# olsonanl/signature_kmers

Measured on AMD Instinct MI355X. Metric: k-mers/sec (extract+hash+count) at 1/2/4/8 GPUs; achieved HBM GB/s %, higher is better.
Workload: dtype u8

## Files before the change

### include/skm.h

```cpp
#ifndef SKM_H
#define SKM_H

#include <stddef.h>
#include <stdint.h>

#ifdef __cplusplus
extern "C" {
#endif

#define SKM_OK 0
#define SKM_E_ARG -1
#define SKM_E_HIP -2
#define SKM_E_OOM -3
#define SKM_E_IO -4
#define SKM_E_COMM -5
#define SKM_E_STATE -6

#define SKM_UNDEFINED_FUNCTION 0xFFFFu

typedef struct skm_stored_kmer_data {
    uint16_t avg_from_end;
    uint16_t function_index;
    uint16_t mean;
    uint16_t median;
// ... 50 lines not shown
int skm_build_prepare(skm_build* b);
int skm_build_run(skm_build* b);
int skm_build_last_timings(skm_build* b, float* ms, int cap);
int skm_build_set_kernel_timing(skm_build* b, int enable, const char* only);
int skm_build_kernel_timings(skm_build* b, char* names, size_t names_cap, float* ms, uint64_t* launches, int cap);
int skm_build_counters(skm_build* b, uint64_t* out, int cap);
typedef struct skm_transport {
    void* ctx;
    int (*alltoallv)(void* ctx, const void* send, const uint64_t* scnt, const uint64_t* soff, void* recv,
                     const uint64_t* rcnt, const uint64_t* roff);
    int (*allreduce)(void* ctx, void* data, uint64_t count, int op);
    int (*allgatherv)(void* ctx, const void* send, void* recv, const uint64_t* bytes_per_rank);
} skm_transport;
int skm_build_set_transport(skm_build* b, const skm_transport* tp);
int skm_debug_exchange_plan(const skm_transport* tp, int rank, int world, uint32_t nb1, const uint64_t* bucket_starts,
                            uint64_t* recv_off, uint64_t* recv_cnt, uint64_t* vstart);
int skm_debug_transport_check(const skm_transport* tp, int rank, int world);

int skm_build_set_option(skm_build* b, const char* name, int64_t value);
int skm_build_debug_stamps(skm_build* b, int enable, uint64_t* out, int cap);
int skm_build_debug_jobs(skm_build* b, uint32_t* out, int cap);
int skm_build_debug_overflow(skm_build* b, uint32_t* out, int cap);
int skm_build_debug_front(skm_build* b, uint64_t* out, int cap);
int skm_build_debug_pass_windows(skm_build* b, uint64_t* out, int cap);
int skm_debug_chain_bench(uint32_t n, uint32_t njobs, int mode, float* ms);
int skm_debug_chain_eval(const uint32_t* samples, uint32_t n, int mode, double* median, double* var);
int skm_debug_div_check(uint64_t nm, uint32_t per, uint64_t* mismatches);
int skm_build_finish(skm_build* b, skm_kept* out);
int skm_build_finish_slice(skm_build* b, int slice_bits, uint32_t slice, skm_kept* out);
int skm_build_signature_flags(skm_build* b, uint8_t* out, uint64_t cap);
void skm_kept_free(skm_kept* k);
void skm_build_destroy(skm_build* b);

int skm_comm_unique_id(uint8_t id[128]);
int skm_build_set_comm(skm_build* b, const uint8_t id[128]);
int skm_build_group_run(skm_build* const* bs, int n);

typedef struct skm_db skm_db;

int skm_db_open(skm_db** out, const char* mph_path, const char* dat_path, int device);
int skm_db_open_mem(skm_db** out, const uint8_t* mph, size_t mph_len, const uint8_t* dat,
                    size_t dat_len, int device);
int skm_db_open_kept(skm_db** out, const uint64_t* keys, const skm_stored_kmer_data* data, size_t n, int device);

typedef struct skm_kept_db_opts {
    uint32_t load_pct;
// ... 188 lines not shown
```

### signature_kmers_amd/__init__.py

```python
from __future__ import annotations

import ctypes as C
import os
from dataclasses import dataclass

import numpy as np

__all__ = [
    "SkmError", "lib", "K", "UNDEFINED_FUNCTION", "STORED_DTYPE", "CALL_DTYPE",
    "SignatureBuilder", "KeptKmers", "CmphKmerDb", "FunctionCaller", "mph_build",
    "kmer_to_str", "str_to_kmer", "keys_from_strings", "device_count", "MatrixDistance", "SeqIdMap",
    "matrix_tile_rows", "KeptKmerDb", "DeviceKeptKmerDb", "kept_db_plan", "kept_slot",
]

K = 8
UNDEFINED_FUNCTION = 0xFFFF
_HERE = os.path.dirname(os.path.abspath(__file__))
LIB_PATH = os.environ.get("SKM_LIB_PATH") or os.path.join(_HERE, "libskm.so")

STORED_DTYPE = np.dtype([("avg_from_end", "<u2"), ("function_index", "<u2"), ("mean", "<u2"),
                         ("median", "<u2"), ("var", "<u2")])
CALL_DTYPE = np.dtype([("start", "<u4"), ("end", "<u4"), ("count", "<i4"), ("function_index", "<u2"),
                       ("pad", "<u2"), ("protein_length_median", "<u4"),
                       ("protein_length_med_avg_dev", "<f4")])
# ... 86 lines not shown
    "skm_version": (C.c_char_p, []),
    "skm_device_count": (C.c_int, [C.POINTER(C.c_int)]),
    "skm_device_mem_info": (C.c_int, [C.c_int, C.POINTER(C.c_uint64), C.POINTER(C.c_uint64)]),
    "skm_build_create": (C.c_int, [C.POINTER(_P), C.POINTER(C.c_int), C.c_int, C.POINTER(_BuildOpts)]),
    "skm_build_add_batch": (C.c_int, [_P, _P, _P, _P, _P, _P, C.c_size_t]),
    "skm_build_prepare": (C.c_int, [_P]),
    "skm_build_run": (C.c_int, [_P]),
    "skm_build_last_timings": (C.c_int, [_P, C.POINTER(C.c_float), C.c_int]),
    "skm_build_set_kernel_timing": (C.c_int, [_P, C.c_int, C.c_char_p]),
    "skm_build_kernel_timings": (C.c_int, [_P, C.c_char_p, C.c_size_t, C.POINTER(C.c_float), C.POINTER(C.c_uint64),
                                           C.c_int]),
    "skm_build_finish": (C.c_int, [_P, C.POINTER(_Kept)]),
    "skm_build_finish_slice": (C.c_int, [_P, C.c_int, C.c_uint32, C.POINTER(_Kept)]),
    "skm_build_signature_flags": (C.c_int, [_P, _P, C.c_uint64]),
    "skm_build_set_option": (C.c_int, [_P, C.c_char_p, C.c_int64]),
    "skm_build_set_transport": (C.c_int, [_P, C.POINTER(_Transport)]),
    "skm_debug_exchange_plan": (C.c_int, [C.POINTER(_Transport), C.c_int, C.c_int, C.c_uint32, _P, _P, _P, _P]),
    "skm_debug_transport_check": (C.c_int, [C.POINTER(_Transport), C.c_int, C.c_int]),
    "skm_build_counters": (C.c_int, [_P, C.POINTER(C.c_uint64), C.c_int]),
    "skm_build_reserve": (C.c_int, [_P, C.c_uint64, C.c_uint64]),
    "skm_build_debug_jobs": (C.c_int, [_P, C.POINTER(C.c_uint32), C.c_int]),
    "skm_build_debug_overflow": (C.c_int, [_P, C.POINTER(C.c_uint32), C.c_int]),
    "skm_build_debug_front": (C.c_int, [_P, C.POINTER(C.c_uint64), C.c_int]),
    "skm_build_debug_pass_windows": (C.c_int, [_P, C.POINTER(C.c_uint64), C.c_int]),
    "skm_debug_chain_bench": (C.c_int, [C.c_uint32, C.c_uint32, C.c_int, C.POINTER(C.c_float)]),
    "skm_debug_chain_eval": (C.c_int, [_P, C.c_uint32, C.c_int, C.POINTER(C.c_double), C.POINTER(C.c_double)]),
    "skm_build_debug_stamps": (C.c_int, [_P, C.c_int, C.POINTER(C.c_uint64), C.c_int]),
    "skm_kept_free": (None, [C.POINTER(_Kept)]),
    "skm_build_destroy": (None, [_P]),
    "skm_comm_unique_id": (C.c_int, [_P]),
    "skm_build_set_comm": (C.c_int, [_P, _P]),
    "skm_build_group_run": (C.c_int, [C.POINTER(_P), C.c_int]),
    "skm_debug_div_check": (C.c_int, [C.c_uint64, C.c_uint32, C.POINTER(C.c_uint64)]),
    "skm_db_open": (C.c_int, [C.POINTER(_P), C.c_char_p, C.c_char_p, C.c_int]),
    "skm_db_open_mem": (C.c_int, [C.POINTER(_P), _P, C.c_size_t, _P, C.c_size_t, C.c_int]),
    "skm_db_open_kept": (C.c_int, [C.POINTER(_P), _P, _P, C.c_size_t, C.c_int]),
    "skm_build_kept_db": (C.c_int, [_P, C.POINTER(_KeptDbOpts), C.POINTER(_P)]),
    "skm_kept_db_plan": (C.c_int, [C.c_uint64, C.POINTER(_KeptDbOpts), C.POINTER(C.c_uint64), C.POINTER(C.c_uint64)]),
    "skm_debug_kept_slot": (C.c_int, [C.c_uint64, C.c_uint64, C.POINTER(C.c_uint64)]),
    "skm_build_mph_db": (C.c_int, [_P, C.POINTER(_MphDbOpts), C.POINTER(_P), C.c_void_p]),
    "skm_mph_db_plan": (C.c_int, [C.c_uint64, C.POINTER(C.c_uint64)]),
    "skm_build_write_final_kmers": (C.c_int, [_P, C.c_char_p, C.POINTER(_FinalKmersStats)]),
    "skm_build_stats": (C.c_int, [_P, C.POINTER(_Kept)]),
    "skm_final_kmers_info": (C.c_int, [C.POINTER(C.c_uint32)]),
    "skm_debug_final_kmers_host": (C.c_int, [_P, _P, C.c_size_t, _P, C.c_size_t, C.POINTER(C.c_uint64)]),
    "skm_db_lookup_fm": (C.c_int, [_P, _P, C.c_size_t, _P]),
# ... 245 lines not shown
                 "free_after_prepare", "recs_rot", "overflow_light_subbuckets", "overflow_light_elements",
                 "groupby_tasks", "groupby_batches"]
        return {names[i]: int(v[i]) for i in range(n)}

    def debug_jobs(self, k: int = 64) -> list:
        v = (C.c_uint32 * k)()
        _check(lib().skm_build_debug_jobs(self._h, v, k))
        return [int(x) for x in v]

    def debug_overflow(self, k: int = 4096) -> list:
        v = (C.c_uint32 * k)()
        n = lib().skm_build_debug_overflow(self._h, v, k)
        return [int(x) for x in v[:min(max(n, 0), k)]]

    def debug_front(self) -> dict:
        names = ["rp", "sel_wg", "sel_span", "emit_g", "pf_span", "pf_nwg", "nwg", "span", "pass_bits",
                 "owner_bits", "b1_bits"]
        v = (C.c_uint64 * len(names))()
        n = lib().skm_build_debug_front(self._h, v, len(names))
        _check(min(n, 0))
        assert n == len(names), n
        return {names[i]: int(v[i]) for i in range(n)}

    def debug_pass_windows(self) -> list:
        v = (C.c_uint64 * 64)()
        n = lib().skm_build_debug_pass_windows(self._h, v, 64)
        _check(min(n, 0))
        return [int(x) for x in v[:n]]

    def debug_stamps(self, enable: bool) -> list:
        v = (C.c_uint64 * 32)()
        _check(lib().skm_build_debug_stamps(self._h, 1 if enable else 0, v, 32))
        return [int(x) for x in v]

    def finish(self) -> KeptKmers:
        k = _Kept()
        _check(lib().skm_build_finish(self._h, C.byref(k)))
        return self._kept(k)

    def finish_slice(self, slice_bits: int, slice_: int) -> KeptKmers:
        k = _Kept()
        _check(lib().skm_build_finish_slice(self._h, int(slice_bits), int(slice_), C.byref(k)))
        return self._kept(k)

    def signature_flags(self) -> np.ndarray:
        n = self.counters()["sequences"]
# ... 824 lines not shown
```

### signature_kmers_amd/csrc/skm_build.hip

```cpp
#include <fcntl.h>
#include <hip/hip_runtime.h>
#include <unistd.h>

#include <algorithm>
#include <cerrno>
#include <type_traits>
#include <chrono>
#include <cmath>
#include <cstdio>
#include <cstdlib>
#include <cstring>
#include <deque>
#include <memory>
#include <numeric>
#include <string>
#include <thread>
#include <vector>

#include "skm_common.h"
#include "skm_keptdb.h"
#include "skm_mphdb.h"
#include "skm_pool.h"
#include "skm_output.h"
#include "skm_util.h"
// ... 1682 lines not shown
                    if (q == j) f = off[j]++;
                s_out[f] = ((uint64_t)(16u * lane + (uint32_t)t) << KEY_BITS) | hs[t];
            }
        }
        wave_sync();
        for (uint32_t j = lane; j < qa[G]; j += 64) {
            uint32_t q = 0;
#pragma unroll
            for (uint32_t k = 1; k < G; ++k) q += j >= qa[k] ? 1u : 0u;
            uint64_t o = 0;
#pragma unroll
            for (uint32_t k = 0; k < G; ++k)
                if (q == k) o = run[k] + (j - qa[k]);
            const uint64_t v = s_out[j];
            if (o < cap) pos[(uint64_t)q * cap + o] = ((t0 - a + (v >> KEY_BITS)) << KEY_BITS) | (v & H43_MASK);
        }
#pragma unroll
        for (uint32_t q = 0; q < G; ++q) run[q] += qa[q + 1] - qa[q];
        wave_sync();
    }
}

constexpr uint32_t PH_THREADS = 512;
__global__ __launch_bounds__(PH_THREADS) void k_pass_hist(const uint64_t* __restrict__ pos, uint64_t cap,
                                                          const unsigned long long* __restrict__ npos, uint32_t NB,
                                                          int rem_bits, uint32_t* __restrict__ hist) {
    extern __shared__ uint32_t s_h[];
    const uint32_t q = blockIdx.y;
    for (uint32_t k = threadIdx.x; k < NB; k += PH_THREADS) s_h[k] = 0;
    __syncthreads();
    const uint64_t n = min((uint64_t)npos[q], cap);
    const uint64_t* p = pos + (uint64_t)q * cap;
    constexpr uint32_t U = 4;
    for (uint64_t j0 = (uint64_t)blockIdx.x * PH_THREADS * U; j0 < n; j0 += (uint64_t)gridDim.x * PH_THREADS * U) {
        uint64_t v[U];
#pragma unroll
        for (uint32_t u = 0; u < U; ++u) {
            const uint64_t j = j0 + u * PH_THREADS + threadIdx.x;
            v[u] = j < n ? p[j] : ~0ull;
        }
#pragma unroll
        for (uint32_t u = 0; u < U; ++u)
            if (v[u] != ~0ull) atomicAdd(&s_h[(uint32_t)((v[u] & H43_MASK) >> rem_bits) & (NB - 1)], 1u);
    }
    __syncthreads();
    uint32_t* hq = hist + (uint64_t)q * NB;
    for (uint32_t k = threadIdx.x; k < NB; k += PH_THREADS)
        if (s_h[k]) atomicAdd(&hq[k], s_h[k]);
}

__global__ __launch_bounds__(EX_THREADS) void k_extract(ExtractArgs X) {
    const uint8_t* __restrict__ res = X.res;
    const uint64_t rp = X.rp, span = X.span;
    extern __shared__ uint32_t s_cnt[];
    const int nbits = X.owner_bits + X.b1_bits;
    const uint32_t NB = 1u << nbits;
    const int rem_bits = KEY_BITS - nbits;
    const uint32_t wg = blockIdx.x;
    for (uint32_t b = threadIdx.x; b < NB; b += blockDim.x) s_cnt[b] = 0u;
    __syncthreads();
    const uint64_t begin = (uint64_t)wg * span;
    const uint64_t end = min(begin + span, rp);
    for (uint64_t base = begin + (uint64_t)threadIdx.x * EX_POS_PER_THREAD; base < end;
         base += (uint64_t)blockDim.x * EX_POS_PER_THREAD) {
        const uint4 v0 = *reinterpret_cast<const uint4*>(res + base);
        const uint4 v1 = *reinterpret_cast<const uint4*>(res + base + 16);
        const uint32_t w[8] = {v0.x, v0.y, v0.z, v0.w, v1.x, v1.y, v1.z, v1.w};
        uint32_t code[24];
// ... 4 lines not shown
            uint32_t cd = residue_code(c);
            valid |= (cd < 40u ? 1u : 0u) << j;
            code[j] = cd < 40u ? cd : 0u;
        }
        uint64_t k = 0;
#pragma unroll
        for (int j = 0; j < 8; ++j) k = k * 40u + code[j];
        constexpr uint64_t P7 = 6553600000000ull / 40u;
#pragma unroll
        for (int t = 0; t < EX_POS_PER_THREAD; ++t) {
            if (t > 0) k = (k - (uint64_t)code[t - 1] * P7) * 40u + code[t + 7];
            const uint64_t p = base + t;
            if (((valid >> t) & 0xFFu) == 0xFFu && p < end) {
                const uint64_t h = mix43(k);
                atomicAdd(&s_cnt[(uint32_t)(h >> rem_bits)], 1u);
            }
        }
    }
    __syncthreads();
    for (uint32_t b = threadIdx.x; b < NB; b += blockDim.x) X.hist[(uint64_t)wg * NB + b] = s_cnt[b];
}

constexpr int SC_ROUND = 4096;
constexpr int SC_L0_BITS = 6;
constexpr int SC_POS = SC_ROUND / EX_THREADS;
constexpr uint64_t SC_SLICE = 65536;

constexpr uint32_t CUR_STRIDE = 16;

template <int R>
struct StageLdsT {
    uint64_t hi[R];
    uint64_t lo[R];
    uint8_t dst[R];
    uint32_t cnt[128];
    uint32_t off[129];
    unsigned long long base[128];
    uint32_t wave[48];
};
using StageLds = StageLdsT<SC_ROUND>;
constexpr int SC_ROUND_HALF = SC_ROUND / 2;

__device__ __forceinline__ uint32_t agg_rank(uint32_t* cnt, uint32_t d, bool v) {
    const uint32_t lane = threadIdx.x & 63u;
    const uint64_t act = __ballot(v);
    if (act == 0) return 0u;
    const uint32_t l0 = (uint32_t)__ffsll((long long)act) - 1u;
// ... 104 lines not shown
        for (int t = 0; t < SC_POS; ++t)
            if ((ok >> t) & 1u) {
                const uint32_t slot = L.off[l0[t]] + rk[t];
                L.hi[slot] = eh[t];
                L.lo[slot] = el[t];
                L.dst[slot] = (uint8_t)l0[t];
            }
        __syncthreads();
        for (uint32_t j = threadIdx.x; j < tot; j += blockDim.x) {
            const uint32_t d = L.dst[j];
            const uint64_t o = L.base[d] + (j - L.off[d]);
            out_hi[o] = L.hi[j];
            out_lo[o] = L.lo[j];
        }
        __syncthreads();
    }
}

template <int R, int MINB>
__global__ __launch_bounds__(EX_THREADS, MINB) void k_extract_stage_pos(ExtractArgs X, const uint64_t* __restrict__ pos,
                                                                        const unsigned long long* __restrict__ np,
                                                                        const uint64_t* __restrict__ sel, uint32_t nrows,
                                                                        uint64_t sel_span,
                                                                        unsigned long long* __restrict__ cur0,
                                                                        uint64_t* __restrict__ out_hi,
                                                                        uint64_t* __restrict__ out_lo) {
    constexpr int SC_POS = R / EX_THREADS;
    const uint64_t n = min((uint64_t)*np, X.pos_cap);
    __shared__ StageLdsT<R> L;
    const int nbits = X.owner_bits + X.b1_bits;
    const uint32_t NB = 1u << nbits;
    const int rem_bits = KEY_BITS - X.pass_bits - nbits;
    const uint64_t rem_mask = (1ull << rem_bits) - 1;
    const int l0_shift = nbits - SC_L0_BITS;
    const uint64_t begin = (uint64_t)blockIdx.x * X.span, end = min(begin + X.span, n);
    uint32_t s = 0xFFFFFFFFu;
    SeqMeta m{};
    uint32_t row = 0;
    {
        const uint64_t j0 = begin + (uint64_t)threadIdx.x * SC_POS;
        uint32_t lo = 0, hi = nrows;
        while (hi - lo > 1) {
            const uint32_t mid = (lo + hi) >> 1;
            if (sel[mid] <= j0)
                lo = mid;
            else
                hi = mid;
        }
        row = lo;
    }
    uint64_t row_end = sel[row + 1];
    uint64_t nxt[SC_POS];
#pragma unroll
    for (int t = 0; t < SC_POS; ++t) {
        const uint64_t j = begin + (uint64_t)threadIdx.x * SC_POS + t;
        nxt[t] = j < end ? pos[j] : ~0ull;
    }
    for (uint64_t base = begin; base < end; base += R) {
        if (threadIdx.x < 128) L.cnt[threadIdx.x] = 0;
        __syncthreads();
        uint64_t ent[SC_POS];
#pragma unroll
        for (int t = 0; t < SC_POS; ++t) ent[t] = nxt[t];
#pragma unroll
        for (int t = 0; t < SC_POS; ++t) {
            const uint64_t j = base + R + (uint64_t)threadIdx.x * SC_POS + t;
            nxt[t] = j < end ? pos[j] : ~0ull;
        }
        uint64_t eh[SC_POS], el[SC_POS];
        uint32_t rk[SC_POS], l0[SC_POS];
#pragma unroll
        for (int t = 0; t < SC_POS; ++t) {
            eh[t] = el[t] = 0;
            rk[t] = l0[t] = 0;
            if (ent[t] != ~0ull) {
                const uint64_t j = base + (uint64_t)threadIdx.x * SC_POS + t;
                while (j >= row_end) row_end = sel[++row + 1];
                const uint64_t p = (uint64_t)row * sel_span + (ent[t] >> KEY_BITS);
                if (s == 0xFFFFFFFFu || p < m.pstart || p > m.pstart + m.len) {
                    s = X.blk2seq[p >> 6];
                    m = X.meta[s];
                }
                while (p > m.pstart + m.len) m = X.meta[++s];
                const uint64_t h = ent[t] & H43_MASK;
                const uint32_t bucket = (uint32_t)(h >> rem_bits) & (NB - 1);
                const uint64_t route = (uint64_t)((uint32_t)(h >> (KEY_BITS - X.pass_bits)) ^ X.pass_id) << rem_bits;
                make_elem((h & rem_mask) | route, X.s_base + s, (uint32_t)(p - m.pstart), m, eh[t], el[t]);
                el[t] = (el[t] & ~0xFFFFull) | bucket;
                l0[t] = bucket >> l0_shift;
            }
        }
#pragma unroll
        for (int t = 0; t < SC_POS; ++t) rk[t] = agg_rank(L.cnt, l0[t], ent[t] != ~0ull);
        __syncthreads();
        const uint32_t tot = stage_reserve(L, 1u << SC_L0_BITS, cur0, 0);
#pragma unroll
        for (int t = 0; t < SC_POS; ++t)
            if (ent[t] != ~0ull) {
                const uint32_t slot = L.off[l0[t]] + rk[t];
                L.hi[slot] = eh[t];
                L.lo[slot] = el[t];
                L.dst[slot] = (uint8_t)l0[t];
            }
        __syncthreads();
        for (uint32_t j = threadIdx.x; j < tot; j += blockDim.x) {
            const uint32_t d = L.dst[j];
            const uint64_t o = L.base[d] + (j - L.off[d]);
            out_hi[o] = L.hi[j];
            out_lo[o] = L.lo[j];
        }
        __syncthreads();
    }
}

__global__ void k_stage_init(const uint64_t* __restrict__ bstart, uint32_t NB, int l0_shift,
                             unsigned long long* __restrict__ cur0, unsigned long long* __restrict__ cur1,
                             uint32_t* __restrict__ slice_base) {
    const uint32_t t = blockIdx.x * blockDim.x + threadIdx.x;
    if (t < NB) cur1[(uint64_t)t * CUR_STRIDE] = bstart[t];
    if (blockIdx.x == 0) {
        __shared__ uint32_t s_n[(1 << SC_L0_BITS) + 1];
        const uint32_t n0 = 1u << SC_L0_BITS;
        if (threadIdx.x < n0) {
            const uint64_t a = bstart[(uint64_t)threadIdx.x << l0_shift];
            const uint64_t e = bstart[(uint64_t)(threadIdx.x + 1) << l0_shift];
            cur0[threadIdx.x * CUR_STRIDE] = a;
            s_n[threadIdx.x] = (uint32_t)((e - a + SC_SLICE - 1) / SC_SLICE);
        }
        __syncthreads();
        if (threadIdx.x == 0) {
            uint32_t acc = 0;
            for (uint32_t b = 0; b < n0; ++b) {
                slice_base[b] = acc;
                acc += s_n[b];
            }
// ... 972 lines not shown
    const uint64_t thr = 2 * (total / max(nb, 1u));
    const uint32_t per = (nb + blockDim.x - 1) / blockDim.x;
    const uint32_t b0 = min(nb, threadIdx.x * per), b1 = min(nb, b0 + per);
    uint32_t loc = 0;
    for (uint32_t b = b0; b < b1; ++b) loc += bstart[b + 1] - bstart[b] > thr ? 1u : 0u;
    uint32_t nbig;
    uint32_t pos = wg_exclusive_scan(loc, s_wave, nbig);
    uint32_t sp = b0 - pos;
    for (uint32_t b = b0; b < b1; ++b) {
        if (bstart[b + 1] - bstart[b] > thr)
            order[pos++] = b;
        else
            order[nbig + sp++] = b;
    }
    if (threadIdx.x == 0) order[nb] = nbig;
}

constexpr uint32_t PS_CUR0 = (1u << SC_L0_BITS) * CUR_STRIDE, PS_SLICES = 80;

__global__ __launch_bounds__(1024) void k_pass_starts(const uint32_t* __restrict__ histg, uint32_t NB, int l0_shift,
                                                      uint32_t set0, uint64_t* __restrict__ bstart,
                                                      unsigned long long* __restrict__ cur0,
                                                      unsigned long long* __restrict__ cur1,
                                                      uint32_t* __restrict__ slice_base, uint32_t* __restrict__ order) {
    __shared__ uint32_t s_wave[48];
    __shared__ uint32_t s_n[(1 << SC_L0_BITS) + 1];
    const uint32_t c = set0 + blockIdx.x;
    const uint32_t* hist = histg + (uint64_t)blockIdx.x * NB;
    bstart += (uint64_t)c * (NB + 1);
    cur0 += (uint64_t)c * PS_CUR0;
    cur1 += (uint64_t)c * NB * CUR_STRIDE;
    slice_base += (uint64_t)c * PS_SLICES;
    const uint32_t per = (NB + blockDim.x - 1) / blockDim.x;
    const uint32_t b0 = min(NB, threadIdx.x * per), b1 = min(NB, b0 + per);
    uint32_t loc = 0;
    for (uint32_t b = b0; b < b1; ++b) loc += hist[b];
    uint32_t total;
    uint32_t run = wg_exclusive_scan(loc, s_wave, total);
    for (uint32_t b = b0; b < b1; ++b) {
        bstart[b] = run;
        cur1[(uint64_t)b * CUR_STRIDE] = run;
        run += hist[b];
    }
    if (threadIdx.x == 0) bstart[NB] = total;
    __syncthreads();
    const uint32_t n0 = 1u << SC_L0_BITS;
    if (threadIdx.x < n0) {
        const uint64_t a = bstart[(uint64_t)threadIdx.x << l0_shift];
        const uint64_t e = bstart[(uint64_t)(threadIdx.x + 1) << l0_shift];
        cur0[threadIdx.x * CUR_STRIDE] = a;
        s_n[threadIdx.x] = (uint32_t)((e - a + SC_SLICE - 1) / SC_SLICE);
    }
    __syncthreads();
    if (threadIdx.x == 0) {
        uint32_t acc = 0;
        for (uint32_t b = 0; b < n0; ++b) {
            slice_base[b] = acc;
            acc += s_n[b];
        }
        slice_base[n0] = acc;
    }
    if (!order) return;
    order += (uint64_t)c * (NB + 1);
    const uint64_t thr = 2 * ((uint64_t)total / max(NB, 1u));
    loc = 0;
    for (uint32_t b = b0; b < b1; ++b) loc += hist[b] > thr ? 1u : 0u;
    uint32_t nbig;
    uint32_t pos = wg_exclusive_scan(loc, s_wave, nbig);
    uint32_t sp = b0 - pos;
    for (uint32_t b = b0; b < b1; ++b) {
        if (hist[b] > thr)
            order[pos++] = b;
        else
            order[nbig + sp++] = b;
    }
    if (threadIdx.x == 0) order[NB] = nbig;
}

constexpr uint32_t PT_ROUND = 2048, PT_THREADS = BP_THREADS;

__device__ __noinline__ void copy_small_bucket(const uint64_t* __restrict__ hi, const uint64_t* __restrict__ lo,
                                               uint64_t* __restrict__ out_hi, uint64_t* __restrict__ out_lo, uint32_t n) {
    for (uint32_t j = threadIdx.x; j < n; j += blockDim.x) {
// ... 1539 lines not shown
    HandoffStats handoff;
    std::vector<uint32_t> h_keep;
    std::vector<uint64_t> h_cum;
    double add_s = 0, add_pack_s = 0, add_wait_s = 0, prep_upload_s = 0, prep_plan_s = 0, prep_rest_s = 0;
    uint64_t n_windows = 0;
    bool seqid_strict = true;
    bool prepared = false, ran = false;
    bool work_released = false;

    DevBuf d_res, d_meta, d_blk2seq, d_glen;
    uint64_t rp = 0;
    uint32_t nseq = 0;
    int world = 1, rank = 0;
    int owner_bits = 0, b1_bits = 12;
    uint32_t s_base = 0;
    uint32_t n_total = 0;
    std::vector<uint32_t> g_seqid;
    bool g_strict = true;
    DevBuf d_hist, d_offs, d_partial, d_rbbase, d_bstart32, d_bstart, d_owner_start;
    DevBuf d_recs_hi, d_recs_lo, d_tmp_hi, d_tmp_lo;
    DevBuf d_stg_hi, d_stg_lo;
    DevBuf d_part_order;
    DevBuf d_cur0, d_cur1, d_slices;
    DevBuf d_flagbits;
    DevBuf d_keys, d_data, d_ctr, d_flags, d_dfunc, d_swf, d_ovf, d_ovf_hi, d_ovf_lo, d_ovf_heads, d_ovf_job, d_ovf_fm;
    DevBuf d_jobs, d_lens, d_stamps, d_big_desc, d_big_out;
    uint64_t big_cap = 0, n_big = 0, big_kept = 0;
    bool stamps = false;
    uint32_t n_cus = 0;
    uint64_t jobs_cap = 0, lens_cap = 0, n_jobs = 0, n_lens = 0;
    uint32_t n_overflow = 0, n_overflow_last = 0;
    uint32_t nwg = 0;
    uint64_t span = 0;
    uint64_t n_kept = 0;
    uint64_t ovf_cap = 0;

    DevBuf d_rhi, d_rlo;
    DevBuf d_cnt_send, d_cnt_recv;
    DevBuf d_seg_start, d_seg_len, d_vstart;
    std::vector<uint64_t> xs_send, xs_recv;
    DevBuf d_xs;
    uint64_t n_local_max = 0;
    uint64_t n_local = 0;
    uint64_t cap_local = 0;

#if defined(SKM_WITH_RCCL)
// ... 560 lines not shown
    b->ovf_cap = c / CAP + NB1 + 16;
    b->jobs_cap = c / 3 + 16;
    b->lens_cap = c + 16;
    b->d_jobs.ensure(sizeof(Job) * b->jobs_cap);
    b->d_lens.ensure(sizeof(uint32_t) * b->lens_cap);
    b->d_ovf.ensure(sizeof(OvfEntry) * b->ovf_cap);
    b->big_cap = c / 65 + 64;
    b->d_big_desc.ensure(16 * b->big_cap);
    b->d_big_out.ensure(sizeof(BigOut) * b->big_cap);
    b->cap_local = c;
}

inline uint32_t pass_copies(const skm_build* b) { return b->pass_bits ? 2u * b->emit_g : 1u; }
inline uint32_t pass_copy(const skm_build* b, uint32_t pass) {
    return b->pass_bits ? ((pass / b->emit_g) & 1u) * b->emit_g + pass % b->emit_g : 0u;
}
void ensure_pass_copies(skm_build* b) {
    const uint64_t NB = 1ull << (b->owner_bits + b->b1_bits), nc = pass_copies(b);
    b->d_bstart.ensure(sizeof(uint64_t) * (NB + 1) * nc);
    b->d_cur0.ensure(8ull * PS_CUR0 * nc);
    b->d_cur1.ensure(8ull * NB * CUR_STRIDE * nc);
    b->d_slices.ensure(4ull * PS_SLICES * nc);
    b->d_part_order.ensure(4ull * (NB + 1) * nc);
}

void size_local(skm_build* b) {
    const uint64_t W = std::max<uint64_t>(b->pass_max, 1);
    b->d_recs_hi.ensure(8 * W);
    b->d_recs_lo.ensure(8 * W);
    if (b->pass_bits > 0) {
        const uint32_t NB = 1u << (b->owner_bits + b->b1_bits);
        const uint32_t P = 1u << b->pass_bits;
        const uint32_t eg = b->tune.emit_group > 0 ? (uint32_t)b->tune.emit_group : 4u;
        b->emit_g = std::max<uint32_t>(1, std::min<uint32_t>(P, eg));
        b->d_posg.ensure(8 * W * b->emit_g);
        b->d_ids.ensure(((b->rp + 15) & ~15ull) + 64);
        SKM_HIP(hipMemsetAsync(b->d_ids.p, 0xFF, ((b->rp + 15) & ~15ull) + 64, b->stream));
        b->d_histg.ensure(sizeof(uint32_t) * (uint64_t)NB * b->emit_g);
        b->d_npos.ensure(8ull * P);
        const uint64_t rmax = (1ull << REL_BITS) - 16;
        b->sel_wg = (uint32_t)std::max<uint64_t>(SEL_WG, ceil_div(std::max<uint64_t>(b->rp, 1), rmax));
        b->d_selrows.ensure(4ull * b->sel_wg * P);
        b->d_seloff.ensure(8ull * P * (b->sel_wg + 1));
        b->sel_span = ceil_div(ceil_div(std::max<uint64_t>(b->rp, 1), b->sel_wg), 16) * 16;
        SKM_CHECK(b->sel_span < (1ull << REL_BITS), SKM_E_STATE, "pass entry row span exceeds REL_BITS");
        const uint64_t stage_wg = b->tune.stage_round == 1 ? 4ull * EX_MAX_WG : EX_MAX_WG;
// ... 292 lines not shown
    for (auto* b : bs) b->prep_rest_s = std::chrono::duration<double>(clk::now() - t2).count();
}

void emit_group(skm_build* b, uint32_t g, hipStream_t st) {
    const uint32_t G = b->emit_g;
    const uint32_t NB = 1u << (b->owner_bits + b->b1_bits);
    const int rem_bits = KEY_BITS - b->pass_bits - b->owner_bits - b->b1_bits;
    const uint64_t cap = std::max<uint64_t>(b->pass_max, 1);
#define SKM_EMIT(GG)                                                                                                    \
    SKM_LAUNCH_AS(b, "k_pass_emit", k_pass_emit<GG>, dim3(b->sel_wg), dim3(EMIT_THREADS), 0, st, b->d_res.as<uint8_t>(), \
                  b->d_ids.as<uint8_t>(), b->rp, g * G, b->sel_span, b->d_seloff.as<uint64_t>(), b->sel_wg, \
                  b->d_posg.as<uint64_t>(), cap)
    if (G == 16)
        SKM_EMIT(16);
    else if (G == 8)
        SKM_EMIT(8);
    else if (G == 4)
        SKM_EMIT(4);
    else if (G == 2)
        SKM_EMIT(2);
    else
        SKM_EMIT(1);
#undef SKM_EMIT
    SKM_HIP(hipMemsetAsync(b->d_histg.p, 0, sizeof(uint32_t) * NB * G, st));
    SKM_LAUNCH(b, k_pass_hist, dim3(256, G), dim3(PH_THREADS), 4u * NB, st, b->d_posg.as<uint64_t>(), cap,
               b->d_npos.as<unsigned long long>() + (uint64_t)g * G, NB, rem_bits, b->d_histg.as<uint32_t>());
    SKM_LAUNCH(b, k_pass_starts, dim3(G), dim3(1024), 0, st, b->d_histg.as<uint32_t>(), NB,
               b->owner_bits + b->b1_bits - SC_L0_BITS, (g & 1u) * G, b->d_bstart.as<uint64_t>(),
               b->d_cur0.as<unsigned long long>(), b->d_cur1.as<unsigned long long>(), b->d_slices.as<uint32_t>(),
               b->world == 1 && b->tune.part_order ? b->d_part_order.as<uint32_t>() : nullptr);
    SKM_HIP(hipGetLastError());
    if (st != b->stream) SKM_HIP(hipEventRecord(b->ev_emit, st));
}

inline uint32_t pass_par(const skm_build* b, uint32_t pass) { return tail_async_on(b) ? pass & 1u : 0u; }
inline unsigned long long* pass_ctr(skm_build* b, uint32_t pass) {
    return b->d_ctr.as<unsigned long long>() + 32 + 32 * pass_par(b, pass);
}
inline uint64_t* pass_hi(skm_build* b, uint32_t pass) { return (pass_par(b, pass) ? b->d_stg_hi : b->d_tmp_hi).as<uint64_t>(); }
inline uint64_t* pass_lo(skm_build* b, uint32_t pass) { return (pass_par(b, pass) ? b->d_stg_lo : b->d_tmp_lo).as<uint64_t>(); }

void join_tail_par(skm_build* b, uint32_t par) {
    if (!b->tail_pending[par]) return;
    SKM_HIP(hipStreamWaitEvent(b->stream, b->ev_tail_done[par], 0));
    b->tail_pending[par] = false;
}
void join_tail(skm_build* b) {
    join_tail_par(b, 0);
    join_tail_par(b, 1);
}

void phase_extract(skm_build* b, uint32_t pass) {
    hipStream_t st = b->stream;
// ... 25 lines not shown
        const uint32_t G = b->emit_g, q = pass % G;
        if (q == 0) {
            if (b->emit_q == (int64_t)(pass / G))
                SKM_HIP(hipStreamWaitEvent(st, b->ev_emit, 0));
            else
                emit_group(b, pass / G, st);
            b->emit_q = -1;
        }
        X.hist = b->d_histg.as<uint32_t>() + (uint64_t)q * NB;
        X.span = b->pf_span;
        nwg = b->pf_nwg;
        hist_rows = 1;
        (void)lds_cnt;
    } else {
        SKM_LAUNCH(b, k_extract, dim3(nwg), dim3(EX_THREADS), lds_cnt, st, X);
    }
    SKM_HIP(hipGetLastError());
    SKM_HIP(hipEventRecord(b->ev[1], st));
    const uint32_t pc = pass_copy(b, pass);
    uint64_t* bstart = b->d_bstart.as<uint64_t>() + (uint64_t)pc * (NB + 1);
    unsigned long long* cur0 = b->d_cur0.as<unsigned long long>() + (uint64_t)pc * PS_CUR0;
    unsigned long long* cur1 = b->d_cur1.as<unsigned long long>() + (uint64_t)pc * NB * CUR_STRIDE;
    uint32_t* slices = b->d_slices.as<uint32_t>() + (uint64_t)pc * PS_SLICES;
    if (!b->pass_bits) {
        const uint32_t nrb = (uint32_t)ceil_div(hist_rows, SCAN_ROWS);
        dim3 gsc((NB + 255) / 256, nrb);
        SKM_LAUNCH(b, k_colsum, gsc, dim3(256), 0, st, X.hist, hist_rows, NB, b->d_partial.as<uint32_t>());
        SKM_LAUNCH(b, k_bstart, dim3(1), dim3(1024), 0, st, b->d_partial.as<uint32_t>(), nrb, NB, b->b1_bits,
                           b->d_rbbase.as<uint32_t>(), b->d_bstart32.as<uint32_t>(), b->d_owner_start.as<uint64_t>(), nowners);
        SKM_LAUNCH(b, k_coloffs, gsc, dim3(256), 0, st, X.hist, b->d_rbbase.as<uint32_t>(), hist_rows,
                           NB, b->d_offs.as<uint32_t>());
        SKM_LAUNCH(b, k_abs_starts, dim3((NB + 1 + 255) / 256), dim3(256), 0, st, b->d_bstart32.as<uint32_t>(),
                           b->d_owner_start.as<uint64_t>(), NB, b->b1_bits, nowners, bstart);
        SKM_HIP(hipGetLastError());
    }
    SKM_HIP(hipEventRecord(b->ev[2], st));
    if (!b->pass_bits) {
        SKM_LAUNCH(b, k_stage_init, dim3((NB + 255) / 256), dim3(256), 0, st, bstart, NB, nbits - SC_L0_BITS, cur0, cur1,
                   slices);
    }
    uint64_t* stg_hi = pass_hi(b, pass);
    uint64_t* stg_lo = pass_lo(b, pass);
    SKM_HIP(hipEventRecord(b->ev[13], st));
    join_tail_par(b, pass_par(b, pass));
    SKM_HIP(hipEventRecord(b->ev[14], st));
    if (b->pass_bits && b->tune.stage_round == 1)
        SKM_LAUNCH_AS(b, "k_extract_stage_pos", (k_extract_stage_pos<SC_ROUND_HALF, 4>), dim3(nwg), dim3(EX_THREADS), 0, st, X,
                   b->d_posg.as<uint64_t>() + (uint64_t)(pass % b->emit_g) * std::max<uint64_t>(b->pass_max, 1),
                   b->d_npos.as<unsigned long long>() + pass,
                   b->d_seloff.as<uint64_t>() + (uint64_t)pass * (b->sel_wg + 1), b->sel_wg, b->sel_span,
                   cur0, stg_hi, stg_lo);
    else if (b->pass_bits)
        SKM_LAUNCH_AS(b, "k_extract_stage_pos", (k_extract_stage_pos<SC_ROUND, 2>), dim3(nwg), dim3(EX_THREADS), 0, st, X,
                   b->d_posg.as<uint64_t>() + (uint64_t)(pass % b->emit_g) * std::max<uint64_t>(b->pass_max, 1),
                   b->d_npos.as<unsigned long long>() + pass,
                   b->d_seloff.as<uint64_t>() + (uint64_t)pass * (b->sel_wg + 1), b->sel_wg, b->sel_span,
                   cur0, stg_hi, stg_lo);
    else
        SKM_LAUNCH(b, k_extract_stage, dim3(nwg), dim3(EX_THREADS), 0, st, X, cur0, stg_hi, stg_lo);
    const uint32_t nsl = (uint32_t)(ceil_div(b->pass_max, SC_SLICE) + (1u << SC_L0_BITS));
    SKM_LAUNCH(b, k_split_stage, dim3(nsl), dim3(EX_THREADS), 0, st, stg_hi,
                       stg_lo, bstart, nbits, slices, cur1, b->d_recs_hi.as<uint64_t>(), b->d_recs_lo.as<uint64_t>());
    SKM_HIP(hipGetLastError());
    SKM_HIP(hipEventRecord(b->ev[3], st));
}

void exchange(const Ranks& bs, uint32_t pass) {
    const int W = bs[0]->world;
    const uint32_t NB1 = 1u << bs[0]->b1_bits;
    const uint32_t NB = NB1 * (uint32_t)W;
    A2A cx, ex_hi, ex_lo;
    for (auto* b : bs) {
        b->d_cnt_send.ensure(4ull * NB);
        b->d_cnt_recv.ensure(4ull * NB);
        SKM_LAUNCH(b, k_send_counts, dim3((NB + 255) / 256), dim3(256), 0, b->stream,
                   b->d_bstart.as<uint64_t>() + (uint64_t)pass_copy(b, pass) * ((1ull << (b->owner_bits + b->b1_bits)) + 1), NB, NB1,
                   (uint32_t)W, b->d_xs.as<unsigned long long>() + (uint64_t)pass * W, b->d_run.as<unsigned long long>(),
                   b->d_cnt_send.as<uint32_t>());
        cx.send.push_back(b->d_cnt_send.as<uint8_t>());
        cx.recv.push_back(b->d_cnt_recv.as<uint8_t>());
// ... 1183 lines not shown
    for (int i = 0; i < cap; ++i) out[i] = (uint32_t)i < n ? e[i].n : 0u;
    return (int)n;
}

int skm_build_debug_front(skm_build* b, uint64_t* out, int cap) {
    if (!b || !out) return SKM_E_ARG;
    if (!b->ran) return SKM_E_STATE;
    const bool passes = b->pass_bits > 0;
    const uint64_t v[11] = {b->rp,
                            passes ? b->sel_wg : 0ull,
                            passes ? b->sel_span : 0ull,
                            passes ? b->emit_g : 0ull,
                            passes ? b->pf_span : 0ull,
                            passes ? b->pf_nwg : 0ull,
                            b->nwg,
                            b->span,
                            (uint64_t)b->pass_bits,
                            (uint64_t)b->owner_bits,
                            (uint64_t)b->b1_bits};
    for (int i = 0; i < cap && i < 11; ++i) out[i] = v[i];
    return 11;
}

int skm_build_debug_pass_windows(skm_build* b, uint64_t* out, int cap) {
    if (!b || !out) return SKM_E_ARG;
    if (!b->ran) return SKM_E_STATE;
    if (hipSetDevice(b->device) != hipSuccess || hipDeviceSynchronize() != hipSuccess) return SKM_E_HIP;
    const uint32_t P = 1u << b->pass_bits;
    std::vector<uint64_t> n(P, b->pass_max);
    if (b->pass_bits) {
        if (!b->d_npos.p || b->d_npos.bytes < 8ull * P) return SKM_E_STATE;
        if (hipMemcpy(n.data(), b->d_npos.p, 8ull * P, hipMemcpyDeviceToHost) != hipSuccess) return SKM_E_HIP;
    }
    for (int i = 0; i < cap && (uint32_t)i < P; ++i) out[i] = n[i];
    return (int)P;
}

int skm_debug_chain_bench(uint32_t n, uint32_t njobs, int mode, float* ms) {
    SKM_API_BEGIN
    SKM_CHECK(ms && n && njobs, SKM_E_ARG, "bad argument");
    std::vector<uint32_t> lens((size_t)n * njobs);
    uint32_t x = 12345;
    for (auto& v : lens) {
        x = x * 1664525u + 1013904223u;
        v = 240 + (x >> 16) % 121;
    }
// ... 337 lines not shown
    }
    out->distinct_signatures = total;
    out->n_seqs_with_signature = ctr[2];
    out->n_windows = b->n_windows;
    out->n_records = b->n_local;
    SKM_API_END
}

int skm_build_signature_flags(skm_build* b, uint8_t* out, uint64_t cap) {
    SKM_API_BEGIN
    SKM_CHECK(b && out, SKM_E_ARG, "null argument");
    SKM_CHECK(b->ran, SKM_E_STATE, "no completed run");
    SKM_HIP(hipSetDevice(b->device));
    const uint64_t n = std::min<uint64_t>(cap, b->n_total);
    if (n) SKM_HIP(hipMemcpy(out, b->d_flags.p, n, hipMemcpyDeviceToHost));
    SKM_API_END
}

static void release_work(skm_build* b) {
    SKM_HIP(hipDeviceSynchronize());
    DevBuf* work[] = {
        &b->d_res, &b->d_meta, &b->d_blk2seq, &b->d_glen, &b->d_hist, &b->d_offs, &b->d_partial, &b->d_rbbase,
        &b->d_bstart32, &b->d_bstart, &b->d_owner_start, &b->d_recs_hi, &b->d_recs_lo, &b->d_tmp_hi, &b->d_tmp_lo,
        &b->d_stg_hi, &b->d_stg_lo, &b->d_part_order, &b->d_cur0, &b->d_cur1, &b->d_slices, &b->d_flagbits,
        &b->d_ovf, &b->d_ovf_hi, &b->d_ovf_lo, &b->d_ovf_heads, &b->d_ovf_job, &b->d_ovf_fm, &b->d_jobs,
        &b->d_lens, &b->d_stamps, &b->d_big_desc, &b->d_big_out, &b->d_rhi, &b->d_rlo, &b->d_cnt_send, &b->d_cnt_recv,
        &b->d_seg_start, &b->d_seg_len, &b->d_vstart, &b->d_xs, &b->d_hv_keys, &b->d_hv_rec, &b->d_hv_len, &b->d_hv_s0,
        &b->d_hv_s1, &b->d_sub_tab, &b->d_jobs2, &b->d_jobs3, &b->d_ids, &b->d_bloom, &b->d_posg, &b->d_histg,
        &b->d_npos, &b->d_selrows, &b->d_seloff, &b->d_gstat, &b->d_long_arena, &b->d_long_jobs, &b->d_ovf2, &b->d_plan,
        &b->d_run};
    for (DevBuf* d : work) d->release();
    for (ChainSet* cs : {&b->cs_main, &b->cs_ovf, &b->cs_ovf3})
        for (DevBuf* d : {&cs->hist, &cs->offs, &cs->sorted, &cs->long_off}) d->release();
    for (auto* q : {&b->gsamples, &b->gjobs, &b->gcount})
        for (DevBuf& d : *q) d.release();
    b->work_released = true;
}

int skm_build_kept_db(skm_build* b, const skm_kept_db_opts* opts, skm_db** out) {
    SKM_API_BEGIN
    SKM_CHECK(b && out, SKM_E_ARG, "null argument");
    *out = nullptr;
    SKM_CHECK(b->world == 1, SKM_E_STATE,
              "skm_build_kept_db needs world_size 1: the kept set of a multi-rank build is sharded over the ranks");
    (void)kept_db_slots(0, opts);
    SKM_HIP(hipSetDevice(b->device));
    if (!b->prepared || !b->ran) run_ranks(Ranks{b});
// ... 129 lines not shown
```

Baseline: 12.12 billion.

## Precompute per-workgroup stage offsets to replace atomic cursor reservation in pass staging

```diff
diff --git a/include/skm.h b/include/skm.h
--- a/include/skm.h
+++ b/include/skm.h
@@ -96,6 +96,7 @@
 int skm_build_debug_jobs(skm_build* b, uint32_t* out, int cap);
 int skm_build_debug_overflow(skm_build* b, uint32_t* out, int cap);
 int skm_build_debug_front(skm_build* b, uint64_t* out, int cap);
+int skm_build_debug_stage_starts(skm_build* b, uint32_t pass, uint64_t* out, int cap);
 int skm_build_debug_pass_windows(skm_build* b, uint64_t* out, int cap);
 int skm_debug_chain_bench(uint32_t n, uint32_t njobs, int mode, float* ms);
 int skm_debug_chain_eval(const uint32_t* samples, uint32_t n, int mode, double* median, double* var);
diff --git a/signature_kmers_amd/__init__.py b/signature_kmers_amd/__init__.py
--- a/signature_kmers_amd/__init__.py
+++ b/signature_kmers_amd/__init__.py
@@ -132,6 +132,7 @@
     "skm_build_debug_jobs": (C.c_int, [_P, C.POINTER(C.c_uint32), C.c_int]),
     "skm_build_debug_overflow": (C.c_int, [_P, C.POINTER(C.c_uint32), C.c_int]),
     "skm_build_debug_front": (C.c_int, [_P, C.POINTER(C.c_uint64), C.c_int]),
+    "skm_build_debug_stage_starts": (C.c_int, [_P, C.c_uint32, C.POINTER(C.c_uint64), C.c_int]),
     "skm_build_debug_pass_windows": (C.c_int, [_P, C.POINTER(C.c_uint64), C.c_int]),
     "skm_debug_chain_bench": (C.c_int, [C.c_uint32, C.c_uint32, C.c_int, C.POINTER(C.c_float)]),
     "skm_debug_chain_eval": (C.c_int, [_P, C.c_uint32, C.c_int, C.POINTER(C.c_double), C.POINTER(C.c_double)]),
@@ -423,6 +424,14 @@
         assert n == len(names), n
         return {names[i]: int(v[i]) for i in range(n)}
 
+    def debug_stage_starts(self, pass_id: int) -> np.ndarray:
+        rows = self.debug_front()["pf_nwg"] + 1
+        out = np.zeros(rows * 64, dtype=np.uint64)
+        n = lib().skm_build_debug_stage_starts(self._h, pass_id, out.ctypes.data_as(C.POINTER(C.c_uint64)), out.size)
+        _check(min(n, 0))
+        assert n == out.size, (n, out.size)
+        return out.reshape(rows, 64)
+
     def debug_pass_windows(self) -> list:
         v = (C.c_uint64 * 64)()
         n = lib().skm_build_debug_pass_windows(self._h, v, 64)
diff --git a/signature_kmers_amd/csrc/skm_build.hip b/signature_kmers_amd/csrc/skm_build.hip
--- a/signature_kmers_amd/csrc/skm_build.hip
+++ b/signature_kmers_amd/csrc/skm_build.hip
@@ -1728,28 +1728,52 @@
 }
 
 constexpr uint32_t PH_THREADS = 512;
+constexpr int SC_L0_BITS = 6;
 __global__ __launch_bounds__(PH_THREADS) void k_pass_hist(const uint64_t* __restrict__ pos, uint64_t cap,
                                                           const unsigned long long* __restrict__ npos, uint32_t NB,
-                                                          int rem_bits, uint32_t* __restrict__ hist) {
+                                                          int rem_bits, uint32_t* __restrict__ hist, uint64_t span,
+                                                          uint32_t nwg, int l0_shift, uint32_t* __restrict__ cnt0) {
     extern __shared__ uint32_t s_h[];
+    __shared__ uint32_t s_prev[1 << SC_L0_BITS];
     const uint32_t q = blockIdx.y;
     for (uint32_t k = threadIdx.x; k < NB; k += PH_THREADS) s_h[k] = 0;
+    if (threadIdx.x < (1u << SC_L0_BITS)) s_prev[threadIdx.x] = 0;
     __syncthreads();
     const uint64_t n = min((uint64_t)npos[q], cap);
     const uint64_t* p = pos + (uint64_t)q * cap;
+    uint32_t* cq = cnt0 + (uint64_t)q * nwg * (1u << SC_L0_BITS);
     constexpr uint32_t U = 4;
-    for (uint64_t j0 = (uint64_t)blockIdx.x * PH_THREADS * U; j0 < n; j0 += (uint64_t)gridDim.x * PH_THREADS * U) {
-        uint64_t v[U];
-#pragma unroll
-        for (uint32_t u = 0; u < U; ++u) {
-            const uint64_t j = j0 + u * PH_THREADS + threadIdx.x;
-            v[u] = j < n ? p[j] : ~0ull;
-        }
-#pragma unroll
-        for (uint32_t u = 0; u < U; ++u)
-            if (v[u] != ~0ull) atomicAdd(&s_h[(uint32_t)((v[u] & H43_MASK) >> rem_bits) & (NB - 1)], 1u);
-    }
-    __syncthreads();
+    constexpr uint32_t GT = PH_THREADS >> SC_L0_BITS;
+    const uint32_t gsz = 1u << l0_shift, gd = threadIdx.x / GT, gs = threadIdx.x % GT;
+    for (uint32_t w = blockIdx.x; w < nwg; w += gridDim.x) {
+        const uint64_t a = (uint64_t)w * span, e = min(a + span, n);
+        if (a >= n) {
+            if (threadIdx.x < (1u << SC_L0_BITS)) cq[(uint64_t)w * (1u << SC_L0_BITS) + threadIdx.x] = 0;
+            continue;
+        }
+        for (uint64_t j0 = a; j0 < e; j0 += PH_THREADS * U) {
+            uint64_t v[U];
+#pragma unroll
+            for (uint32_t u = 0; u < U; ++u) {
+                const uint64_t j = j0 + u * PH_THREADS + threadIdx.x;
+                v[u] = j < e ? p[j] : ~0ull;
+            }
+#pragma unroll
+            for (uint32_t u = 0; u < U; ++u)
+                if (v[u] != ~0ull) atomicAdd(&s_h[(uint32_t)((v[u] & H43_MASK) >> rem_bits) & (NB - 1)], 1u);
+        }
+        __syncthreads();
+        uint32_t sum = 0;
+        for (uint32_t k = gs; k < gsz; k += GT) sum += s_h[gd * gsz + k];
+        sum += xshfl<1>(sum);
+        sum += xshfl<2>(sum);
+        sum += xshfl<4>(sum);
+        if (gs == 0) {
+            cq[(uint64_t)w * (1u << SC_L0_BITS) + gd] = sum - s_prev[gd];
+            s_prev[gd] = sum;
+        }
+        __syncthreads();
+    }
     uint32_t* hq = hist + (uint64_t)q * NB;
     for (uint32_t k = threadIdx.x; k < NB; k += PH_THREADS)
         if (s_h[k]) atomicAdd(&hq[k], s_h[k]);
@@ -1800,7 +1824,6 @@
 }
 
 constexpr int SC_ROUND = 4096;
-constexpr int SC_L0_BITS = 6;
 constexpr int SC_POS = SC_ROUND / EX_THREADS;
 constexpr uint64_t SC_SLICE = 65536;
 
@@ -1951,12 +1974,20 @@
                                                                         const unsigned long long* __restrict__ np,
                                                                         const uint64_t* __restrict__ sel, uint32_t nrows,
                                                                         uint64_t sel_span,
-                                                                        unsigned long long* __restrict__ cur0,
+                                                                        const uint32_t* __restrict__ wstart,
+                                                                        unsigned long long* __restrict__ run,
                                                                         uint64_t* __restrict__ out_hi,
                                                                         uint64_t* __restrict__ out_lo) {
     constexpr int SC_POS = R / EX_THREADS;
+    constexpr uint32_t N0 = 1u << SC_L0_BITS;
     const uint64_t n = min((uint64_t)*np, X.pos_cap);
     __shared__ StageLdsT<R> L;
+    __shared__ uint64_t s_cur[N0];
+    __shared__ uint32_t s_end[N0];
+    if (threadIdx.x < N0) {
+        s_cur[threadIdx.x] = wstart[(uint64_t)blockIdx.x * N0 + threadIdx.x];
+        s_end[threadIdx.x] = wstart[(uint64_t)(blockIdx.x + 1) * N0 + threadIdx.x];
+    }
     const int nbits = X.owner_bits + X.b1_bits;
     const uint32_t NB = 1u << nbits;
     const int rem_bits = KEY_BITS - X.pass_bits - nbits;
@@ -1985,9 +2016,9 @@
         const uint64_t j = begin + (uint64_t)threadIdx.x * SC_POS + t;
         nxt[t] = j < end ? pos[j] : ~0ull;
     }
+    if (threadIdx.x < N0) L.cnt[threadIdx.x] = 0;
+    __syncthreads();
     for (uint64_t base = begin; base < end; base += R) {
-        if (threadIdx.x < 128) L.cnt[threadIdx.x] = 0;
-        __syncthreads();
         uint64_t ent[SC_POS];
 #pragma unroll
         for (int t = 0; t < SC_POS; ++t) ent[t] = nxt[t];
@@ -2022,7 +2053,19 @@
 #pragma unroll
         for (int t = 0; t < SC_POS; ++t) rk[t] = agg_rank(L.cnt, l0[t], ent[t] != ~0ull);
         __syncthreads();
-        const uint32_t tot = stage_reserve(L, 1u << SC_L0_BITS, cur0, 0);
+        if (threadIdx.x < N0) {
+            const uint32_t c = L.cnt[threadIdx.x];
+            L.cnt[threadIdx.x] = 0;
+            const uint32_t inc = wave_incl_scan(c);
+            L.off[threadIdx.x] = inc - c;
+            if (threadIdx.x == N0 - 1) L.off[N0] = inc;
+            const uint64_t cur = s_cur[threadIdx.x], e = s_end[threadIdx.x];
+            const uint64_t fit = cur < e ? min((uint64_t)c, e - cur) : 0ull;
+            L.base[threadIdx.x] = (cur & 0xFFFFFFFFull) | (fit << 32);
+            s_cur[threadIdx.x] = cur + c;
+        }
+        __syncthreads();
+        const uint32_t tot = L.off[N0];
 #pragma unroll
         for (int t = 0; t < SC_POS; ++t)
             if (ent[t] != ~0ull) {
@@ -2034,12 +2077,17 @@
         __syncthreads();
         for (uint32_t j = threadIdx.x; j < tot; j += blockDim.x) {
             const uint32_t d = L.dst[j];
-            const uint64_t o = L.base[d] + (j - L.off[d]);
-            out_hi[o] = L.hi[j];
-            out_lo[o] = L.lo[j];
-        }
-        __syncthreads();
-    }
+            const uint64_t bf = L.base[d];
+            const uint32_t r = j - L.off[d];
+            if (r < (uint32_t)(bf >> 32)) {
+                const uint64_t o = (bf & 0xFFFFFFFFull) + r;
+                out_hi[o] = L.hi[j];
+                out_lo[o] = L.lo[j];
+            }
+        }
+    }
+    if (threadIdx.x < N0 && s_cur[threadIdx.x] != s_end[threadIdx.x])
+        atomicOr(&run[RUN_FLAGS], (unsigned long long)RUN_F_CAP);
 }
 
 __global__ void k_stage_init(const uint64_t* __restrict__ bstart, uint32_t NB, int l0_shift,
@@ -3058,9 +3106,13 @@
                                                       uint32_t set0, uint64_t* __restrict__ bstart,
                                                       unsigned long long* __restrict__ cur0,
                                                       unsigned long long* __restrict__ cur1,
-                                                      uint32_t* __restrict__ slice_base, uint32_t* __restrict__ order) {
+                                                      uint32_t* __restrict__ slice_base, uint32_t* __restrict__ order,
+                                                      const uint32_t* __restrict__ cnt0, uint32_t nwg,
+                                                      uint32_t* __restrict__ wstart) {
     __shared__ uint32_t s_wave[48];
     __shared__ uint32_t s_n[(1 << SC_L0_BITS) + 1];
+    __shared__ uint32_t s_start[1 << SC_L0_BITS];
+    __shared__ uint32_t s_part[16 << SC_L0_BITS];
     const uint32_t c = set0 + blockIdx.x;
     const uint32_t* hist = histg + (uint64_t)blockIdx.x * NB;
     bstart += (uint64_t)c * (NB + 1);
@@ -3085,6 +3137,7 @@
         const uint64_t a = bstart[(uint64_t)threadIdx.x << l0_shift];
         const uint64_t e = bstart[(uint64_t)(threadIdx.x + 1) << l0_shift];
         cur0[threadIdx.x * CUR_STRIDE] = a;
+        s_start[threadIdx.x] = (uint32_t)a;
         s_n[threadIdx.x] = (uint32_t)((e - a + SC_SLICE - 1) / SC_SLICE);
     }
     __syncthreads();
@@ -3095,6 +3148,24 @@
             acc += s_n[b];
         }
         slice_base[n0] = acc;
+    }
+    {
+        cnt0 += (uint64_t)blockIdx.x * nwg * n0;
+        wstart += (uint64_t)c * (nwg + 1) * n0;
+        const uint32_t d = threadIdx.x & (n0 - 1), part = threadIdx.x >> SC_L0_BITS, parts = blockDim.x >> SC_L0_BITS;
+        const uint32_t per_w = (nwg + parts - 1) / parts;
+        const uint32_t w0 = min(nwg, part * per_w), w1 = min(nwg, w0 + per_w);
+        uint32_t sum = 0;
+        for (uint32_t w = w0; w < w1; ++w) sum += cnt0[(uint64_t)w * n0 + d];
+        s_part[part * n0 + d] = sum;
+        __syncthreads();
+        uint32_t at = s_start[d];
+        for (uint32_t k = 0; k < part; ++k) at += s_part[k * n0 + d];
+        for (uint32_t w = w0; w < w1; ++w) {
+            wstart[(uint64_t)w * n0 + d] = at;
+            at += cnt0[(uint64_t)w * n0 + d];
+        }
+        if (part == parts - 1) wstart[(uint64_t)nwg * n0 + d] = at;
     }
     if (!order) return;
     order += (uint64_t)c * (NB + 1);
@@ -4680,6 +4751,7 @@
     DevBuf d_stg_hi, d_stg_lo;
     DevBuf d_part_order;
     DevBuf d_cur0, d_cur1, d_slices;
+    DevBuf d_cnt0, d_wstart;
     DevBuf d_flagbits;
     DevBuf d_keys, d_data, d_ctr, d_flags, d_dfunc, d_swf, d_ovf, d_ovf_hi, d_ovf_lo, d_ovf_heads, d_ovf_job, d_ovf_fm;
     DevBuf d_jobs, d_lens, d_stamps, d_big_desc, d_big_out;
@@ -5286,6 +5358,10 @@
     b->d_cur1.ensure(8ull * NB * CUR_STRIDE * nc);
     b->d_slices.ensure(4ull * PS_SLICES * nc);
     b->d_part_order.ensure(4ull * (NB + 1) * nc);
+    if (b->pass_bits) {
+        b->d_wstart.ensure(4ull * ((uint64_t)b->pf_nwg + 1) * (1u << SC_L0_BITS) * nc);
+        b->d_cnt0.ensure(4ull * b->pf_nwg * (1u << SC_L0_BITS) * b->emit_g);
+    }
 }
 
 void size_local(skm_build* b) {
@@ -5624,13 +5700,16 @@
     else
         SKM_EMIT(1);
 #undef SKM_EMIT
+    const int l0_shift = b->owner_bits + b->b1_bits - SC_L0_BITS;
     SKM_HIP(hipMemsetAsync(b->d_histg.p, 0, sizeof(uint32_t) * NB * G, st));
     SKM_LAUNCH(b, k_pass_hist, dim3(256, G), dim3(PH_THREADS), 4u * NB, st, b->d_posg.as<uint64_t>(), cap,
-               b->d_npos.as<unsigned long long>() + (uint64_t)g * G, NB, rem_bits, b->d_histg.as<uint32_t>());
-    SKM_LAUNCH(b, k_pass_starts, dim3(G), dim3(1024), 0, st, b->d_histg.as<uint32_t>(), NB,
-               b->owner_bits + b->b1_bits - SC_L0_BITS, (g & 1u) * G, b->d_bstart.as<uint64_t>(),
-               b->d_cur0.as<unsigned long long>(), b->d_cur1.as<unsigned long long>(), b->d_slices.as<uint32_t>(),
-               b->world == 1 && b->tune.part_order ? b->d_part_order.as<uint32_t>() : nullptr);
+               b->d_npos.as<unsigned long long>() + (uint64_t)g * G, NB, rem_bits, b->d_histg.as<uint32_t>(),
+               b->pf_span, b->pf_nwg, l0_shift, b->d_cnt0.as<uint32_t>());
+    SKM_LAUNCH(b, k_pass_starts, dim3(G), dim3(1024), 0, st, b->d_histg.as<uint32_t>(), NB, l0_shift, (g & 1u) * G,
+               b->d_bstart.as<uint64_t>(), b->d_cur0.as<unsigned long long>(), b->d_cur1.as<unsigned long long>(),
+               b->d_slices.as<uint32_t>(),
+               b->world == 1 && b->tune.part_order ? b->d_part_order.as<uint32_t>() : nullptr,
+               b->d_cnt0.as<uint32_t>(), b->pf_nwg, b->d_wstart.as<uint32_t>());
     SKM_HIP(hipGetLastError());
     if (st != b->stream) SKM_HIP(hipEventRecord(b->ev_emit, st));
 }
@@ -5702,6 +5781,8 @@
     unsigned long long* cur0 = b->d_cur0.as<unsigned long long>() + (uint64_t)pc * PS_CUR0;
     unsigned long long* cur1 = b->d_cur1.as<unsigned long long>() + (uint64_t)pc * NB * CUR_STRIDE;
     uint32_t* slices = b->d_slices.as<uint32_t>() + (uint64_t)pc * PS_SLICES;
+    const uint32_t* wstart =
+        b->pass_bits ? b->d_wstart.as<uint32_t>() + (uint64_t)pc * (((uint64_t)b->pf_nwg + 1) << SC_L0_BITS) : nullptr;
     if (!b->pass_bits) {
         const uint32_t nrb = (uint32_t)ceil_div(hist_rows, SCAN_ROWS);
         dim3 gsc((NB + 255) / 256, nrb);
@@ -5729,13 +5810,13 @@
                    b->d_posg.as<uint64_t>() + (uint64_t)(pass % b->emit_g) * std::max<uint64_t>(b->pass_max, 1),
                    b->d_npos.as<unsigned long long>() + pass,
                    b->d_seloff.as<uint64_t>() + (uint64_t)pass * (b->sel_wg + 1), b->sel_wg, b->sel_span,
-                   cur0, stg_hi, stg_lo);
+                   wstart, b->d_run.as<unsigned long long>(), stg_hi, stg_lo);
     else if (b->pass_bits)
         SKM_LAUNCH_AS(b, "k_extract_stage_pos", (k_extract_stage_pos<SC_ROUND, 2>), dim3(nwg), dim3(EX_THREADS), 0, st, X,
                    b->d_posg.as<uint64_t>() + (uint64_t)(pass % b->emit_g) * std::max<uint64_t>(b->pass_max, 1),
                    b->d_npos.as<unsigned long long>() + pass,
                    b->d_seloff.as<uint64_t>() + (uint64_t)pass * (b->sel_wg + 1), b->sel_wg, b->sel_span,
-                   cur0, stg_hi, stg_lo);
+                   wstart, b->d_run.as<unsigned long long>(), stg_hi, stg_lo);
     else
         SKM_LAUNCH(b, k_extract_stage, dim3(nwg), dim3(EX_THREADS), 0, st, X, cur0, stg_hi, stg_lo);
     const uint32_t nsl = (uint32_t)(ceil_div(b->pass_max, SC_SLICE) + (1u << SC_L0_BITS));
@@ -6965,6 +7046,21 @@
     return 11;
 }
 
+int skm_build_debug_stage_starts(skm_build* b, uint32_t pass, uint64_t* out, int cap) {
+    if (!b || !out) return SKM_E_ARG;
+    if (!b->ran || !b->pass_bits || b->work_released || !b->d_wstart.p) return SKM_E_STATE;
+    const uint32_t P = 1u << b->pass_bits;
+    if (pass >= P || pass / b->emit_g != (P - 1) / b->emit_g) return SKM_E_ARG;
+    if (hipSetDevice(b->device) != hipSuccess || hipDeviceSynchronize() != hipSuccess) return SKM_E_HIP;
+    const uint64_t n = ((uint64_t)b->pf_nwg + 1) << SC_L0_BITS;
+    std::vector<uint32_t> v(n);
+    if (hipMemcpy(v.data(), b->d_wstart.as<uint32_t>() + (uint64_t)pass_copy(b, pass) * n, 4 * n, hipMemcpyDeviceToHost) !=
+        hipSuccess)
+        return SKM_E_HIP;
+    for (uint64_t i = 0; i < n && i < (uint64_t)std::max(cap, 0); ++i) out[i] = v[i];
+    return (int)n;
+}
+
 int skm_build_debug_pass_windows(skm_build* b, uint64_t* out, int cap) {
     if (!b || !out) return SKM_E_ARG;
     if (!b->ran) return SKM_E_STATE;
@@ -7348,7 +7444,8 @@
     DevBuf* work[] = {
         &b->d_res, &b->d_meta, &b->d_blk2seq, &b->d_glen, &b->d_hist, &b->d_offs, &b->d_partial, &b->d_rbbase,
         &b->d_bstart32, &b->d_bstart, &b->d_owner_start, &b->d_recs_hi, &b->d_recs_lo, &b->d_tmp_hi, &b->d_tmp_lo,
-        &b->d_stg_hi, &b->d_stg_lo, &b->d_part_order, &b->d_cur0, &b->d_cur1, &b->d_slices, &b->d_flagbits,
+        &b->d_stg_hi, &b->d_stg_lo, &b->d_part_order, &b->d_cur0, &b->d_cur1, &b->d_slices, &b->d_cnt0, &b->d_wstart,
+        &b->d_flagbits,
         &b->d_ovf, &b->d_ovf_hi, &b->d_ovf_lo, &b->d_ovf_heads, &b->d_ovf_job, &b->d_ovf_fm, &b->d_jobs,
         &b->d_lens, &b->d_stamps, &b->d_big_desc, &b->d_big_out, &b->d_rhi, &b->d_rlo, &b->d_cnt_send, &b->d_cnt_recv,
         &b->d_seg_start, &b->d_seg_len, &b->d_vstart, &b->d_xs, &b->d_hv_keys, &b->d_hv_rec, &b->d_hv_len, &b->d_hv_s0,
```

New measurement: 12.33 billion (median of 6 runs). 1.02x the previous value.
